# Modalities/modalities

Hardware: AMD Instinct MI355X
Metric: train_tokens_per_s (higher is better)
Workload: dtype bf16; 1 GPU; model=gpt2-2.7b, global_batch=2, micro_batch=2, seq_len=4096, parallelism=dp1_fullshard_hipgraph, num_params=2795276800

## Files before the change

### modalities_amd/ops/adamw.py

```python

from typing import Iterable

import torch

from modalities_amd.ops.backend import hip_ext, hip_available


@torch.no_grad()
def fused_adamw_step(params: list, grads: list, exp_avgs: list, exp_avg_sqs: list,
                     step: int, lr: float, beta1: float, beta2: float,
                     eps: float, weight_decay: float) -> None:
    bc1 = 1.0 - beta1 ** step
    bc2 = 1.0 - beta2 ** step
    if hip_available() and params and params[0].is_cuda:
        hip_ext().fused_adamw(params, grads, exp_avgs, exp_avg_sqs,
                              lr, beta1, beta2, eps, weight_decay, bc1, bc2)
        return
    for p, g, m, v in zip(params, grads, exp_avgs, exp_avg_sqs):
        p.mul_(1.0 - lr * weight_decay)
        m.mul_(beta1).add_(g, alpha=1 - beta1)
        v.mul_(beta2).addcmul_(g, g, value=1 - beta2)
        denom = (v / bc2).sqrt_().add_(eps)
        p.addcdiv_(m, denom, value=-lr / bc1)


@torch.no_grad()
def multi_tensor_l2norm(tensors: Iterable[torch.Tensor]) -> torch.Tensor:
    tensors = [t for t in tensors if t is not None]
    if not tensors:
        return torch.zeros((), dtype=torch.float32)
    if hip_available() and tensors[0].is_cuda:
        return hip_ext().multi_tensor_sqsum(list(tensors)).sqrt()
    acc = torch.zeros((), dtype=torch.float32, device=tensors[0].device)
    for t in tensors:
        acc += t.float().pow(2).sum()
    return acc.sqrt()


@torch.no_grad()
def multi_tensor_scale_(tensors: Iterable[torch.Tensor], scale: torch.Tensor) -> None:
    tensors = [t for t in tensors if t is not None]
    if not tensors:
        return
    if hip_available() and tensors[0].is_cuda and isinstance(scale, torch.Tensor):
        hip_ext().multi_tensor_scale(list(tensors), scale)
        return
    for t in tensors:
        t.mul_(scale.to(t.device) if isinstance(scale, torch.Tensor) else scale)
```

### modalities_amd/ops/csrc/adamw.hip

```cpp
#include <torch/extension.h>
#include <ATen/hip/HIPContext.h>
#include "common.h"

namespace {

__global__ void adamw_masked_kernel(float* __restrict__ p,
                                    const float* __restrict__ g,
                                    float* __restrict__ m,
                                    float* __restrict__ v,
                                    const float* __restrict__ wd_mask,
                                    long n4, float lr, float beta1, float beta2,
                                    float eps, float wd, float bc1, float bc2) {
  const float step_size = lr / bc1;
  const float inv_bc2 = 1.0f / bc2;
  floatx4* p4 = reinterpret_cast<floatx4*>(p);
  const floatx4* g4 = reinterpret_cast<const floatx4*>(g);
  floatx4* m4 = reinterpret_cast<floatx4*>(m);
  floatx4* v4 = reinterpret_cast<floatx4*>(v);
  const floatx4* w4 = reinterpret_cast<const floatx4*>(wd_mask);
  for (long i = blockIdx.x * (long)blockDim.x + threadIdx.x; i < n4;
       i += (long)gridDim.x * blockDim.x) {
    floatx4 pp = p4[i], gg = g4[i], mm = m4[i], vv = v4[i], ww = w4[i];
#pragma unroll
    for (int j = 0; j < 4; ++j) {
      pp[j] *= (1.0f - lr * wd * ww[j]);
      mm[j] = beta1 * mm[j] + (1.0f - beta1) * gg[j];
      vv[j] = beta2 * vv[j] + (1.0f - beta2) * gg[j] * gg[j];
      pp[j] -= step_size * mm[j] / (sqrtf(vv[j] * inv_bc2) + eps);
    }
    p4[i] = pp; m4[i] = mm; v4[i] = vv;
  }
}

__device__ __forceinline__ float bias_correction(float beta, float t) {
  return -expm1f(t * logf(beta));
}

__global__ void adamw_masked_devstep_kernel(float* __restrict__ p,
                                            const float* __restrict__ g,
                                            float* __restrict__ m,
                                            float* __restrict__ v,
                                            const float* __restrict__ wd_mask,
                                            const int* __restrict__ step,
                                            unsigned short* __restrict__ bf16_out,
                                            const float* __restrict__ gscale,
                                            long n4, float lr, float beta1,
                                            float beta2, float eps, float wd) {
  const float gs = gscale ? *gscale : 1.0f;
  const float t = (float)*step;
  const float bc1 = bias_correction(beta1, t);
  const float bc2 = bias_correction(beta2, t);
  const float step_size = lr / bc1;
  const float inv_bc2 = 1.0f / bc2;
  floatx4* p4 = reinterpret_cast<floatx4*>(p);
  const floatx4* g4 = reinterpret_cast<const floatx4*>(g);
  floatx4* m4 = reinterpret_cast<floatx4*>(m);
  floatx4* v4 = reinterpret_cast<floatx4*>(v);
  const floatx4* w4 = reinterpret_cast<const floatx4*>(wd_mask);
  for (long i = blockIdx.x * (long)blockDim.x + threadIdx.x; i < n4;
       i += (long)gridDim.x * blockDim.x) {
    floatx4 pp = p4[i], gg = g4[i], mm = m4[i], vv = v4[i], ww = w4[i];
    shortx4 h;
#pragma unroll
    for (int j = 0; j < 4; ++j) {
      const float gj = gg[j] * gs;
      pp[j] *= (1.0f - lr * wd * ww[j]);
      mm[j] = beta1 * mm[j] + (1.0f - beta1) * gj;
      vv[j] = beta2 * vv[j] + (1.0f - beta2) * gj * gj;
      pp[j] -= step_size * mm[j] / (sqrtf(vv[j] * inv_bc2) + eps);
      h[j] = (short)f32_to_bf16(pp[j]);
    }
    p4[i] = pp; m4[i] = mm; v4[i] = vv;
    reinterpret_cast<shortx4*>(bf16_out)[i] = h;
  }
}

template <int W>
__global__ void adamw_devstep_wide_kernel(float* __restrict__ p,
                                          const float* __restrict__ g,
                                          float* __restrict__ m,
                                          float* __restrict__ v,
                                          const float* __restrict__ wd_mask,
                                          const int* __restrict__ step,
                                          unsigned short* __restrict__ bf16_out,
                                          const float* __restrict__ gscale,
                                          long n4, float lr, float beta1,
                                          float beta2, float eps, float wd) {
  const float gs = gscale ? *gscale : 1.0f;
  const float t = (float)*step;
  const float bc1 = bias_correction(beta1, t);
  const float bc2 = bias_correction(beta2, t);
  const float step_size = lr / bc1;
  const float inv_bc2 = 1.0f / bc2;
  floatx4* p4 = reinterpret_cast<floatx4*>(p);
  const floatx4* g4 = reinterpret_cast<const floatx4*>(g);
  floatx4* m4 = reinterpret_cast<floatx4*>(m);
  floatx4* v4 = reinterpret_cast<floatx4*>(v);
  const floatx4* w4 = reinterpret_cast<const floatx4*>(wd_mask);
  const long stride = (long)gridDim.x * blockDim.x;
  for (long i0 = ((long)blockIdx.x * blockDim.x + threadIdx.x) * W;
       i0 < n4; i0 += stride * W) {
    floatx4 pp[W], gg[W], mm[W], vv[W], ww[W];
    shortx4 h[W];
#pragma unroll
    for (int u = 0; u < W; ++u)
      if (i0 + u < n4) {
        pp[u] = p4[i0 + u]; gg[u] = g4[i0 + u]; mm[u] = m4[i0 + u];
        vv[u] = v4[i0 + u]; ww[u] = w4[i0 + u];
      }
#pragma unroll
    for (int u = 0; u < W; ++u) {
#pragma unroll
      for (int j = 0; j < 4; ++j) {
        const float gj = gg[u][j] * gs;
        pp[u][j] *= (1.0f - lr * wd * ww[u][j]);
        mm[u][j] = beta1 * mm[u][j] + (1.0f - beta1) * gj;
        vv[u][j] = beta2 * vv[u][j] + (1.0f - beta2) * gj * gj;
        pp[u][j] -= step_size * mm[u][j] / (sqrtf(vv[u][j] * inv_bc2) + eps);
        h[u][j] = (short)f32_to_bf16(pp[u][j]);
      }
    }
#pragma unroll
    for (int u = 0; u < W; ++u)
      if (i0 + u < n4) {
        p4[i0 + u] = pp[u]; m4[i0 + u] = mm[u]; v4[i0 + u] = vv[u];
        reinterpret_cast<shortx4*>(bf16_out)[i0 + u] = h[u];
      }
  }
}

__global__ void sqsum_kernel(const float* __restrict__ x, long n4,
                             float* __restrict__ out) {
  __shared__ float scratch[256 / WAVE_SIZE];
  const floatx4* x4 = reinterpret_cast<const floatx4*>(x);
  float acc = 0.f;
  for (long i = blockIdx.x * (long)blockDim.x + threadIdx.x; i < n4;
       i += (long)gridDim.x * blockDim.x) {
    floatx4 v = x4[i];
#pragma unroll
    for (int j = 0; j < 4; ++j) acc += v[j] * v[j];
  }
  acc = block_reduce_sum(acc, scratch);
  if (threadIdx.x == 0) atomicAdd(out, acc);
}

__global__ void scale_kernel(float* __restrict__ x, long n4,
                             const float* __restrict__ scale) {
  const float s = *scale;
  floatx4* x4 = reinterpret_cast<floatx4*>(x);
  for (long i = blockIdx.x * (long)blockDim.x + threadIdx.x; i < n4;
       i += (long)gridDim.x * blockDim.x) {
    floatx4 v = x4[i];
#pragma unroll
    for (int j = 0; j < 4; ++j) v[j] *= s;
    x4[i] = v;
  }
}

int grid_for(long work, int block) {
  long g = (work + block - 1) / block;
  return (int)min(g, (long)(256 * 8));
}

bool f32_like(const torch::Tensor& t, const torch::Tensor& ref) {
  return t.is_cuda() && t.dtype() == torch::kFloat32 && t.is_contiguous()
      && t.numel() == ref.numel() && t.device() == ref.device();
}

}

void fused_adamw_masked(torch::Tensor p, torch::Tensor g, torch::Tensor m,
                        torch::Tensor v, torch::Tensor wd_mask, double lr,
                        double beta1, double beta2, double eps, double wd,
                        double bc1, double bc2) {
  TORCH_CHECK(p.is_cuda() && p.dtype() == torch::kFloat32 && p.is_contiguous());
  TORCH_CHECK(p.numel() % 4 == 0, "flat shard must be divisible by 4");
  TORCH_CHECK(f32_like(g, p) && f32_like(m, p) && f32_like(v, p)
              && f32_like(wd_mask, p),
              "g, m, v, wd_mask must match p (device fp32, contiguous)");
  long n4 = p.numel() / 4;
  auto stream = at::cuda::getCurrentHIPStream();
  hipLaunchKernelGGL(adamw_masked_kernel, dim3(grid_for(n4, 256)), dim3(256), 0,
                     stream, p.data_ptr<float>(), g.data_ptr<float>(),
                     m.data_ptr<float>(), v.data_ptr<float>(),
                     wd_mask.data_ptr<float>(), n4, (float)lr, (float)beta1,
                     (float)beta2, (float)eps, (float)wd, (float)bc1, (float)bc2);
  HIP_CHECK_KERNEL();
}

void fused_adamw_masked_devstep(torch::Tensor p, torch::Tensor g,
                                torch::Tensor m, torch::Tensor v,
                                torch::Tensor wd_mask, torch::Tensor step,
                                torch::Tensor bf16_out,
                                c10::optional<torch::Tensor> gscale, double lr,
                                double beta1, double beta2, double eps,
                                double wd) {
  const float* gs_ptr = nullptr;
  if (gscale.has_value()) {
    TORCH_CHECK(gscale->is_cuda() && gscale->dtype() == torch::kFloat32
                && gscale->numel() == 1, "gscale must be a cuda fp32 scalar");
    gs_ptr = gscale->data_ptr<float>();
  }
  TORCH_CHECK(p.is_cuda() && p.dtype() == torch::kFloat32 && p.is_contiguous());
  TORCH_CHECK(p.numel() % 4 == 0, "flat shard must be divisible by 4");
  TORCH_CHECK(f32_like(g, p) && f32_like(m, p) && f32_like(v, p)
              && f32_like(wd_mask, p),
              "g, m, v, wd_mask must match p (device fp32, contiguous)");
  TORCH_CHECK(step.is_cuda() && step.dtype() == torch::kInt32
              && step.numel() == 1);
  TORCH_CHECK(bf16_out.is_cuda() && bf16_out.dtype() == torch::kBFloat16
              && bf16_out.is_contiguous() && bf16_out.numel() == p.numel());
  long n4 = p.numel() / 4;
  auto stream = at::cuda::getCurrentHIPStream();
  static const int wide = []() {
    const char* e = getenv("MODALITIES_AMD_ADAMW_WIDE");
    return e ? atoi(e) : 1;
  }();
  if (wide >= 4) {
    hipLaunchKernelGGL(adamw_devstep_wide_kernel<4>,
                       dim3(grid_for((n4 + 3) / 4, 256)), dim3(256), 0, stream,
                       p.data_ptr<float>(), g.data_ptr<float>(),
                       m.data_ptr<float>(), v.data_ptr<float>(),
                       wd_mask.data_ptr<float>(), step.data_ptr<int>(),
                       (unsigned short*)bf16_out.data_ptr(), gs_ptr, n4,
                       (float)lr, (float)beta1, (float)beta2, (float)eps,
                       (float)wd);
  } else if (wide >= 2) {
    hipLaunchKernelGGL(adamw_devstep_wide_kernel<2>,
                       dim3(grid_for((n4 + 1) / 2, 256)), dim3(256), 0, stream,
                       p.data_ptr<float>(), g.data_ptr<float>(),
                       m.data_ptr<float>(), v.data_ptr<float>(),
                       wd_mask.data_ptr<float>(), step.data_ptr<int>(),
                       (unsigned short*)bf16_out.data_ptr(), gs_ptr, n4,
                       (float)lr, (float)beta1, (float)beta2, (float)eps,
                       (float)wd);
  } else {
    hipLaunchKernelGGL(adamw_masked_devstep_kernel, dim3(grid_for(n4, 256)),
                       dim3(256), 0, stream, p.data_ptr<float>(),
                       g.data_ptr<float>(), m.data_ptr<float>(),
                       v.data_ptr<float>(), wd_mask.data_ptr<float>(),
                       step.data_ptr<int>(),
                       (unsigned short*)bf16_out.data_ptr(), gs_ptr, n4,
                       (float)lr, (float)beta1, (float)beta2, (float)eps,
                       (float)wd);
  }
  HIP_CHECK_KERNEL();
}

void fused_adamw(std::vector<torch::Tensor> ps, std::vector<torch::Tensor> gs,
                 std::vector<torch::Tensor> ms, std::vector<torch::Tensor> vs,
                 double lr, double beta1, double beta2, double eps, double wd,
                 double bc1, double bc2) {
  TORCH_CHECK(gs.size() == ps.size() && ms.size() == ps.size()
              && vs.size() == ps.size(), "fused_adamw: list lengths differ");
  for (size_t i = 0; i < ps.size(); ++i) {
    auto ones = torch::ones_like(ps[i]);
    fused_adamw_masked(ps[i], gs[i], ms[i], vs[i], ones, lr, beta1, beta2, eps,
                       wd, bc1, bc2);
  }
}

torch::Tensor multi_tensor_sqsum(std::vector<torch::Tensor> tensors) {
  TORCH_CHECK(!tensors.empty());
  auto out = torch::zeros({}, tensors[0].options().dtype(torch::kFloat32));
  auto stream = at::cuda::getCurrentHIPStream();
  for (auto& t : tensors) {
    TORCH_CHECK(t.is_cuda() && t.dtype() == torch::kFloat32
                && t.is_contiguous() && t.numel() % 4 == 0);
    long n4 = t.numel() / 4;
    hipLaunchKernelGGL(sqsum_kernel, dim3(grid_for(n4, 256)), dim3(256), 0,
                       stream, t.data_ptr<float>(), n4, out.data_ptr<float>());
    HIP_CHECK_KERNEL();
  }
  return out;
}

void multi_tensor_scale(std::vector<torch::Tensor> tensors, torch::Tensor scale) {
  TORCH_CHECK(scale.is_cuda() && scale.numel() == 1,
              "multi_tensor_scale: scale must be a device scalar");
  for (auto& t : tensors)
    TORCH_CHECK(t.is_cuda() && t.dtype() == torch::kFloat32
                && t.is_contiguous() && t.numel() % 4 == 0,
                "multi_tensor_scale: tensors must be contiguous device fp32 "
                "with numel % 4 == 0");
  auto stream = at::cuda::getCurrentHIPStream();
  auto s = scale.to(torch::kFloat32).contiguous();
  for (auto& t : tensors) {
    long n4 = t.numel() / 4;
    hipLaunchKernelGGL(scale_kernel, dim3(grid_for(n4, 256)), dim3(256), 0,
                       stream, t.data_ptr<float>(), n4, s.data_ptr<float>());
    HIP_CHECK_KERNEL();
  }
}
```

### modalities_amd/ops/csrc/bindings.cpp

```cpp
#include <torch/extension.h>

std::vector<torch::Tensor> rmsnorm_fwd(torch::Tensor x, torch::Tensor w, double eps);
std::vector<torch::Tensor> rmsnorm_bwd(torch::Tensor dy, torch::Tensor x,
                                       torch::Tensor w, torch::Tensor invrms);
std::vector<torch::Tensor> layernorm_fwd(torch::Tensor x, torch::Tensor w,
                                         c10::optional<torch::Tensor> b,
                                         double eps);
std::vector<torch::Tensor> layernorm_bwd(torch::Tensor dy, torch::Tensor x,
                                         torch::Tensor w, torch::Tensor mean,
                                         torch::Tensor rstd, bool has_bias);
long layernorm_max_h();
torch::Tensor rope_fwd(torch::Tensor x, torch::Tensor cos_t, torch::Tensor sin_t,
                       bool neg);
torch::Tensor rope_fwd_slice(torch::Tensor qkv, torch::Tensor cos_t,
                             torch::Tensor sin_t, long col_off, long Hn,
                             long D, bool neg);
void rope_bwd_slice(torch::Tensor dx, torch::Tensor cos_t, torch::Tensor sin_t,
                    torch::Tensor dqkv, long col_off);
torch::Tensor silu_mul_fwd(torch::Tensor g, torch::Tensor u);
std::vector<torch::Tensor> silu_mul_bwd(torch::Tensor dout, torch::Tensor g,
                                        torch::Tensor u);
torch::Tensor silu_mul_joint_fwd(torch::Tensor wv);
torch::Tensor silu_mul_joint_bwd(torch::Tensor dout, torch::Tensor wv);
std::vector<torch::Tensor> cross_entropy_fwd(torch::Tensor logits,
                                             torch::Tensor targets,
                                             long ignore_index);
torch::Tensor cross_entropy_bwd(torch::Tensor logits, torch::Tensor targets,
                                torch::Tensor lse, torch::Tensor scale,
                                long ignore_index);
void fused_adamw_masked(torch::Tensor p, torch::Tensor g, torch::Tensor m,
                        torch::Tensor v, torch::Tensor wd_mask, double lr,
                        double beta1, double beta2, double eps, double wd,
                        double bc1, double bc2);
void fused_adamw_masked_devstep(torch::Tensor p, torch::Tensor g,
                                torch::Tensor m, torch::Tensor v,
                                torch::Tensor wd_mask, torch::Tensor step,
                                torch::Tensor bf16_out,
                                c10::optional<torch::Tensor> gscale, double lr,
                                double beta1, double beta2, double eps,
                                double wd);
void fused_adamw(std::vector<torch::Tensor> ps, std::vector<torch::Tensor> gs,
                 std::vector<torch::Tensor> ms, std::vector<torch::Tensor> vs,
                 double lr, double beta1, double beta2, double eps, double wd,
                 double bc1, double bc2);
torch::Tensor multi_tensor_sqsum(std::vector<torch::Tensor> tensors);
void multi_tensor_scale(std::vector<torch::Tensor> tensors, torch::Tensor scale);
std::vector<torch::Tensor> attn_fwd(torch::Tensor q, torch::Tensor k,
                                    torch::Tensor v, bool causal,
                                    long q_offset);
std::vector<torch::Tensor> attn_bwd(torch::Tensor dout, torch::Tensor q,
                                    torch::Tensor k, torch::Tensor v,
                                    torch::Tensor o, torch::Tensor lse,
                                    bool causal, long q_offset,
                                    c10::optional<torch::Tensor> dlse);
torch::Tensor mfma_probe_32x32x16(torch::Tensor a, torch::Tensor b);
torch::Tensor tr16_probe(long mode);
std::vector<torch::Tensor> attn_fwd_ablate(torch::Tensor q, torch::Tensor k,
                                           torch::Tensor v, long mode);
std::vector<torch::Tensor> attn_bwd_qkvjoint(torch::Tensor dout,
                                             torch::Tensor q, torch::Tensor k,
                                             torch::Tensor v, torch::Tensor o,
                                             torch::Tensor lse, bool causal,
                                             long q_offset, torch::Tensor dqkv,
                                             long dv_col_off);
std::vector<torch::Tensor> attn_bwd_dkdv_ablate(torch::Tensor dout,
                                                torch::Tensor q,
                                                torch::Tensor k,
                                                torch::Tensor v,
                                                torch::Tensor lse,
                                                torch::Tensor delta, long mode);
std::vector<torch::Tensor> attn_fwd2(torch::Tensor q, torch::Tensor k,
                                     torch::Tensor v, bool causal,
                                     long q_offset);
std::vector<torch::Tensor> attn_bwd2(torch::Tensor dout, torch::Tensor q,
                                     torch::Tensor k, torch::Tensor v,
                                     torch::Tensor o, torch::Tensor lse,
                                     bool causal, long q_offset,
                                     c10::optional<torch::Tensor> dlse);
std::vector<torch::Tensor> attn_bwd2_qkvjoint(torch::Tensor dout,
                                              torch::Tensor q, torch::Tensor k,
                                              torch::Tensor v, torch::Tensor o,
                                              torch::Tensor lse, bool causal,
                                              long q_offset, torch::Tensor dqkv,
                                              long dv_col_off);
std::vector<torch::Tensor> attn_fwd2_doc(torch::Tensor q, torch::Tensor k,
                                         torch::Tensor v, bool causal,
                                         long q_offset,
                                         torch::Tensor doc_start);
std::vector<torch::Tensor> attn_bwd2_doc(torch::Tensor dout, torch::Tensor q,
                                         torch::Tensor k, torch::Tensor v,
                                         torch::Tensor o, torch::Tensor lse,
                                         bool causal, long q_offset,
                                         torch::Tensor doc_start,
                                         torch::Tensor doc_end,
                                         c10::optional<torch::Tensor> dlse);
std::vector<torch::Tensor> attn_bwd2_qkvjoint_doc(
    torch::Tensor dout, torch::Tensor q, torch::Tensor k, torch::Tensor v,
    torch::Tensor o, torch::Tensor lse, bool causal, long q_offset,
    torch::Tensor doc_start, torch::Tensor doc_end, torch::Tensor dqkv,
    long dv_col_off);
std::vector<torch::Tensor> decode_attn_fwd(torch::Tensor q,
                                           torch::Tensor k_cache,
                                           torch::Tensor v_cache,
                                           torch::Tensor kv_lens,
                                           long kv_chunk);
long decode_attn_kv_chunk();
long decode_attn_kv_chunk_min();
torch::Tensor decode_rope_append(torch::Tensor q, torch::Tensor k,
                                 torch::Tensor v,
                                 c10::optional<torch::Tensor> cos_t,
                                 c10::optional<torch::Tensor> sin_t,
                                 torch::Tensor pos, torch::Tensor k_cache,
                                 torch::Tensor v_cache);

static int g_attn_impl = [] {
  const char* e = getenv("MA_ATTN_IMPL");
  return e ? atoi(e) : 2;
}();

PYBIND11_MODULE(TORCH_EXTENSION_NAME, m) {
  m.def("rmsnorm_fwd", &rmsnorm_fwd, "RMSNorm forward (K5)");
  m.def("rmsnorm_bwd", &rmsnorm_bwd, "RMSNorm backward (K5)");
  m.def("layernorm_fwd", &layernorm_fwd,
        "LayerNorm forward (K5): (y, mean, rstd); b may be None",
        py::arg("x"), py::arg("w"), py::arg("b"), py::arg("eps"));
  m.def("layernorm_bwd", &layernorm_bwd,
        "LayerNorm backward (K5): (dx, dw, db); db is empty without bias",
        py::arg("dy"), py::arg("x"), py::arg("w"), py::arg("mean"),
        py::arg("rstd"), py::arg("has_bias"));
  m.def("layernorm_max_h", &layernorm_max_h,
        "largest row length the LayerNorm kernels take");
  m.def("rope_fwd", &rope_fwd, "RoPE rotate-half (K4); neg=true => inverse");
  m.def("rope_fwd_slice", &rope_fwd_slice,
        "RoPE a head-block slice of fused QKV into a contiguous [B,T,H,D]");
  m.def("rope_bwd_slice", &rope_bwd_slice,
        "inverse-RoPE a [B,T,H,D] grad into a fused-QKV grad buffer slice");
  m.def("silu_mul_fwd", &silu_mul_fwd, "silu(g)*u forward (K6)");
  m.def("silu_mul_bwd", &silu_mul_bwd, "silu(g)*u backward (K6)");
  m.def("silu_mul_joint_fwd", &silu_mul_joint_fwd,
        "silu/mul over a packed [.., 2H] gate|up tensor (K6 joint)");
  m.def("silu_mul_joint_bwd", &silu_mul_joint_bwd,
        "joint-layout silu/mul backward into one dwv buffer");
  m.def("cross_entropy_fwd", &cross_entropy_fwd, "fused CE forward (K8)");
  m.def("cross_entropy_bwd", &cross_entropy_bwd, "fused CE backward (K8)");
  m.def("fused_adamw_masked", &fused_adamw_masked,
        "AdamW on a flat fp32 shard with per-element wd mask (K9)");
  m.def("fused_adamw", &fused_adamw, "multi-tensor AdamW (K9)");
  m.def("fused_adamw_masked_devstep", &fused_adamw_masked_devstep,
        "AdamW with device-resident step counter (hipGraph-safe)");
  m.def("multi_tensor_sqsum", &multi_tensor_sqsum, "sum of squares (K10)");
  m.def("multi_tensor_scale", &multi_tensor_scale, "in-place scale (K10)");
  m.def("attn_fwd",
        [](torch::Tensor q, torch::Tensor k, torch::Tensor v, bool causal,
           long q_offset) {
          const long D = q.size(3);
          return (g_attn_impl == 2 || D == 80)
              ? attn_fwd2(q, k, v, causal, q_offset)
              : attn_fwd(q, k, v, causal, q_offset);
        },
        "flash attention forward (K1)", py::arg("q"), py::arg("k"),
        py::arg("v"), py::arg("causal"), py::arg("q_offset") = 0);
  m.def("attn_bwd",
        [](torch::Tensor dout, torch::Tensor q, torch::Tensor k,
           torch::Tensor v, torch::Tensor o, torch::Tensor lse, bool causal,
           long q_offset, c10::optional<torch::Tensor> dlse) {
          const long D = q.size(3);
          return (g_attn_impl == 2 || D == 80)
              ? attn_bwd2(dout, q, k, v, o, lse, causal, q_offset, dlse)
              : attn_bwd(dout, q, k, v, o, lse, causal, q_offset, dlse);
        },
        "flash attention backward (K1); dlse = d(loss)/d(lse) fp32 [B,Hq,T] "
        "or None", py::arg("dout"), py::arg("q"),
        py::arg("k"), py::arg("v"), py::arg("o"), py::arg("lse"),
        py::arg("causal"), py::arg("q_offset") = 0,
        py::arg("dlse") = py::none());
  m.def("set_attn_impl", [](long v) { g_attn_impl = (int)v; },
        "select the K1 kernel generation (1 or 2) for A/B");
  m.def("get_attn_impl", []() { return (long)g_attn_impl; });
  m.def("attn_fwd_v1", &attn_fwd, "K1 v1 forward (direct, for A/B)");
  m.def("attn_bwd_v1", &attn_bwd, "K1 v1 backward (direct, for A/B)",
        py::arg("dout"), py::arg("q"), py::arg("k"), py::arg("v"),
        py::arg("o"), py::arg("lse"), py::arg("causal"), py::arg("q_offset"),
        py::arg("dlse") = py::none());
  m.def("attn_fwd_v2", &attn_fwd2, "K1 v2 forward (direct, for A/B)");
  m.def("attn_bwd_v2", &attn_bwd2, "K1 v2 backward (direct, for A/B)",
        py::arg("dout"), py::arg("q"), py::arg("k"), py::arg("v"),
        py::arg("o"), py::arg("lse"), py::arg("causal"), py::arg("q_offset"),
        py::arg("dlse") = py::none());
  m.def("tr16_probe", &tr16_probe, "ds_read_b64_tr_b16 semantics probe");
  m.def("mfma_probe_32x32x16", &mfma_probe_32x32x16,
        "MFMA fragment-layout probe (verification)");
  m.def("attn_fwd_ablate", &attn_fwd_ablate,
        "attention fwd cost-attribution ablation (timing only)");
  m.def("attn_bwd_qkvjoint",
        [](torch::Tensor dout, torch::Tensor q, torch::Tensor k,
           torch::Tensor v, torch::Tensor o, torch::Tensor lse, bool causal,
           long q_offset, torch::Tensor dqkv, long dv_col_off) {
          const long D = q.size(3);
          return (g_attn_impl == 2 || D == 80)
              ? attn_bwd2_qkvjoint(dout, q, k, v, o, lse, causal, q_offset,
                                   dqkv, dv_col_off)
              : attn_bwd_qkvjoint(dout, q, k, v, o, lse, causal, q_offset,
                                  dqkv, dv_col_off);
// ... 73 lines not shown
```

### modalities_amd/optimizers/optimizer_factory.py

```python

from typing import Optional

import torch

from modalities_amd.parallel.fsdp import XGMIShardedModel


class ShardedAdamW(torch.optim.Optimizer):

    def __init__(self, sharded_model: XGMIShardedModel, lr: float = 3e-4,
                 betas: tuple[float, float] = (0.9, 0.95), eps: float = 1e-8,
                 weight_decay: float = 0.1):
        self.sharded_model = sharded_model
        sharded_model._optimizer_consumes_grad_scale = True
        sharded_model._pending_grad_scale = None
        params = [u.master_shard for u in sharded_model.units]
        defaults = dict(lr=lr, betas=betas, eps=eps, weight_decay=weight_decay)
        super().__init__(params, defaults)
        for u in sharded_model.units:
            st = self.state[u.master_shard]
            st["step"] = 0
            st["exp_avg"] = torch.zeros_like(u.master_shard)
            st["exp_avg_sq"] = torch.zeros_like(u.master_shard)
        self._step_dev = None

    @torch.no_grad()
    def step(self, closure=None):
        loss = closure() if closure is not None else None
        group = self.param_groups[0]
        lr, (beta1, beta2) = group["lr"], group["betas"]
        eps, wd = group["eps"], group["weight_decay"]
        from modalities_amd.ops.backend import hip_available, hip_ext
        on_gpu = hip_available() and self.sharded_model.units \
            and self.sharded_model.units[0].master_shard.is_cuda
        if on_gpu:
            if self._step_dev is None:
                start = max((self.state[u.master_shard].get("step", 0)
                             for u in self.sharded_model.units), default=0)
                self._step_dev = torch.tensor(
                    start, dtype=torch.int32,
                    device=self.sharded_model.units[0].master_shard.device)
            self._step_dev += 1
            fresh = [u.grad_fresh for u in self.sharded_model.units]
            if any(fresh) and not all(fresh):
                raise RuntimeError(
                    "fused AdamW devstep: mixed grad_fresh across units "
                    f"({sum(fresh)}/{len(fresh)}) — the shared device step "
                    "counter requires all units to step together")
        gscale = getattr(self.sharded_model, "_pending_grad_scale", None)
        self.sharded_model._pending_grad_scale = None
        for ui, u in enumerate(self.sharded_model.units):
            if not u.grad_fresh:
                continue
            st = self.state[u.master_shard]
            st["step"] += 1
            step = st["step"]
            m, v = st["exp_avg"], st["exp_avg_sq"]
            g = u.grad_shard
            p = u.master_shard
            if on_gpu and u.bf16_shard.dtype == torch.bfloat16:
                hip_ext().fused_adamw_masked_devstep(
                    p, g, m, v, u.wd_mask_shard, self._step_dev,
                    u.bf16_shard, gscale, lr, beta1, beta2, eps, wd)
                if u.full_buf is not None and self.sharded_model.world > 1:
                    u.free_full()
                self.sharded_model.prefetch_unit_gather(ui)
            elif on_gpu:
                if gscale is not None:
                    g = g.mul(gscale)
                bc1 = 1.0 - beta1 ** step
                bc2 = 1.0 - beta2 ** step
                hip_ext().fused_adamw_masked(p, g, m, v, u.wd_mask_shard,
                                             lr, beta1, beta2, eps, wd,
                                             bc1, bc2)
                u.publish_master()
            else:
                if gscale is not None:
                    g = g.mul(gscale)
                bc1 = 1.0 - beta1 ** step
                bc2 = 1.0 - beta2 ** step
                p.mul_(1.0 - lr * wd * u.wd_mask_shard)
                m.mul_(beta1).add_(g, alpha=1 - beta1)
                v.mul_(beta2).addcmul_(g, g, value=1 - beta2)
                denom = (v / bc2).sqrt().add_(eps)
                p.add_(-lr / bc1 * m / denom)
        if on_gpu:
            pass
        else:
            self.sharded_model.publish_master()
            for ui in range(len(self.sharded_model.units)):
                self.sharded_model.prefetch_unit_gather(ui)
        return loss

    def zero_grad(self, set_to_none: bool = True):
        self.sharded_model.zero_grad_shards()


def get_adam_w(wrapped_model, lr: float = 3e-4, betas=(0.9, 0.95), eps: float = 1e-8,
               weight_decay: float = 0.1, weight_decay_groups_excluded=None,
               foreach: Optional[bool] = None, fused: Optional[bool] = None):
    if isinstance(wrapped_model, XGMIShardedModel):
        return ShardedAdamW(wrapped_model, lr=lr, betas=betas, eps=eps,
                            weight_decay=weight_decay)
    decay, no_decay = [], []
    for name, p in wrapped_model.named_parameters():
        if not p.requires_grad:
            continue
        (no_decay if p.ndim < 2 or "norm" in name.lower() or name.endswith(".bias")
         else decay).append(p)
    groups = [{"params": decay, "weight_decay": weight_decay},
              {"params": no_decay, "weight_decay": 0.0}]
    return torch.optim.AdamW(groups, lr=lr, betas=betas, eps=eps,
# ... 2 lines not shown
```

### modalities_amd/parallel/fsdp.py

```python

import re
from contextlib import contextmanager
from typing import Optional

import torch
import torch.distributed as dist
import torch.nn as nn


def _pad_to(n: int, multiple: int) -> int:
    return (n + multiple - 1) // multiple * multiple


class _CommStreams:
    def __init__(self, device: torch.device):
        self.on_gpu = device.type == "cuda"
        self.gather = torch.cuda.Stream(device=device) if self.on_gpu else None
        self.reduce = torch.cuda.Stream(device=device) if self.on_gpu else None

    @contextmanager
    def on(self, stream):
        if self.on_gpu and stream is not None:
            with torch.cuda.stream(stream):
                yield
        else:
            yield


class FlatParamUnit:

    def __init__(self, name: str, modules: list[nn.Module], device: torch.device,
                 group, rank: int, world: int, param_dtype: torch.dtype,
                 no_decay_patterns: Optional[list[str]] = None):
        self.name = name
        self.modules = modules
        self.device = device
        self.group = group
        self.rank = rank
        self.world = world
        self.param_dtype = param_dtype

        seen: dict[int, int] = {}
        self.param_infos: list[tuple[nn.Module, str, nn.Parameter]] = []
        for mod in modules:
            for pname, p in mod.named_parameters(recurse=True):
                if id(p) in seen:
                    continue
                seen[id(p)] = len(self.param_infos)
                self.param_infos.append((mod, pname, p))

        self.shapes = [p.shape for _, _, p in self.param_infos]
        self.numels = [p.numel() for _, _, p in self.param_infos]
        self.offsets = []
        off = 0
        for n in self.numels:
            self.offsets.append(off)
            off += n
        self.total_numel = _pad_to(max(off, 1), max(world, 1) * 64)
        self.shard_numel = self.total_numel // world

        nd_res = [re.compile(pat) for pat in (no_decay_patterns or [])]
        flat_mask = torch.ones(self.total_numel, dtype=torch.float32)
        for (mod, pname, p), offset, numel in zip(self.param_infos, self.offsets,
                                                  self.numels):
            full_name = f"{type(mod).__name__}.{pname}"
            no_decay = p.ndim < 2 or any(r.search(full_name) for r in nd_res)
            if no_decay:
                flat_mask[offset:offset + numel] = 0.0
        s = self.rank * self.shard_numel
        self.wd_mask_shard = flat_mask[s:s + self.shard_numel].to(device)

        self.master_shard = torch.zeros(self.shard_numel, dtype=torch.float32, device=device)
        self.grad_shard = torch.empty(self.shard_numel, dtype=torch.float32, device=device)
        self.grad_fresh = False
        self.bf16_shard = torch.zeros(self.shard_numel, dtype=param_dtype, device=device)
        self.full_buf: Optional[torch.Tensor] = None
        self.grad_full: Optional[torch.Tensor] = None
        self.is_gathered = False
        self.grads_allocated = False
        self.grads_seen = 0
        self._gather_event = None
        self._reduce_event = None


    @torch.no_grad()
    def init_from_materialized(self):
        flat = torch.zeros(self.total_numel, dtype=torch.float32, device=self.device)
        for (_, _, p), off, n in zip(self.param_infos, self.offsets, self.numels):
            flat[off:off + n] = p.detach().float().reshape(-1).to(self.device)
        s = self.rank * self.shard_numel
        self.master_shard.copy_(flat[s:s + self.shard_numel])
        self.bf16_shard.copy_(self.master_shard.to(self.param_dtype))
        del flat
        self._point_params_to(None)

    @torch.no_grad()
    def _point_params_to(self, full_buf: Optional[torch.Tensor]):
        for (_, _, p), off, n, shape in zip(self.param_infos, self.offsets,
                                            self.numels, self.shapes):
            if full_buf is None:
                p.data = torch.empty(0, dtype=self.param_dtype, device=self.device)
            else:
                p.data = full_buf[off:off + n].view(shape)


    def gather(self, streams: _CommStreams):
        if self.is_gathered:
            return
        if self.world == 1:
            self.full_buf = self.bf16_shard
            self.is_gathered = True
            return
        with streams.on(streams.gather):
            if streams.on_gpu:
                streams.gather.wait_stream(torch.cuda.current_stream(self.device))
            self.full_buf = torch.empty(self.total_numel, dtype=self.param_dtype,
                                        device=self.device)
            dist.all_gather_into_tensor(self.full_buf, self.bf16_shard, group=self.group)
            if streams.on_gpu:
                self._gather_event = torch.cuda.Event()
                self._gather_event.record(streams.gather)
        self.is_gathered = True

    def wait_gather(self, streams: _CommStreams):
        if streams.on_gpu and self._gather_event is not None:
            torch.cuda.current_stream(self.device).wait_event(self._gather_event)
            self._gather_event = None
            if self.full_buf is not None and self.full_buf.is_cuda:
                self.full_buf.record_stream(
                    torch.cuda.current_stream(self.device))
        self._point_params_to(self.full_buf)

    @torch.no_grad()
    def free_full(self):
        self._point_params_to(None)
        self.full_buf = None
        self.is_gathered = False


    @torch.no_grad()
    def alloc_grad_views(self):
        if self.grad_full is None:
            self.grad_full = torch.zeros(self.total_numel, dtype=self.param_dtype,
                                         device=self.device)
        for (_, _, p), off, n, shape in zip(self.param_infos, self.offsets,
                                            self.numels, self.shapes):
            p.grad = self.grad_full[off:off + n].view(shape)
        self.grads_allocated = True

    def reduce_scatter_grads(self, streams: _CommStreams):
        gf = self.grad_full
        if gf is None:
            return
        with streams.on(streams.reduce):
            if streams.on_gpu:
                streams.reduce.wait_stream(torch.cuda.current_stream(self.device))
            if self.world > 1:
                backend = dist.get_backend(self.group) if self.group is not None \
                    else dist.get_backend()
                if backend != "gloo":
                    out = torch.empty(self.shard_numel, dtype=self.param_dtype,
                                      device=self.device)
                    dist.reduce_scatter_tensor(out, gf, group=self.group)
                else:
                    dist.all_reduce(gf, group=self.group)
                    s = self.rank * self.shard_numel
                    out = gf[s:s + self.shard_numel]
            else:
                out = gf
            scale = 1.0 / self.world
            if self.grad_fresh:
                self.grad_shard.add_(out, alpha=scale)
            else:
                self.grad_shard.copy_(out)
                if scale != 1.0:
                    self.grad_shard.mul_(scale)
                self.grad_fresh = True
            if streams.on_gpu:
                self._reduce_event = torch.cuda.Event()
                self._reduce_event.record(streams.reduce)
                gf.record_stream(streams.reduce)
        for _, _, p in self.param_infos:
            p.grad = None
        self.grad_full = None
        self.grads_allocated = False

    def wait_reduce(self):
        if self._reduce_event is not None:
            torch.cuda.current_stream(self.device).wait_event(self._reduce_event)
            self._reduce_event = None

    @torch.no_grad()
    def publish_master(self):
        self.bf16_shard.copy_(self.master_shard)
        if self.world > 1 and self.full_buf is not None:
            self.free_full()


class _UnshardBackwardAnchor(torch.autograd.Function):

    @staticmethod
    def forward(ctx, engine, unit_idx, t):
        ctx.engine = engine
        ctx.unit_idx = unit_idx
        return t.view_as(t)

    @staticmethod
    def backward(ctx, grad):
        ctx.engine._pre_backward(ctx.unit_idx)
        return None, None, grad


class XGMIShardedModel(nn.Module):

    def __init__(self, module: nn.Module, device: torch.device,
                 process_group=None, rank: Optional[int] = None,
                 world_size: Optional[int] = None,
                 unit_modules: Optional[list[list[nn.Module]]] = None,
                 param_dtype: torch.dtype = torch.bfloat16,
                 reshard_after_forward: bool = False,
                 no_decay_patterns: Optional[list[str]] = None,
                 replicate_group=None):
        super().__init__()
        self.module = module
        self.device = device
        self.group = process_group
        if world_size is None:
            world_size = dist.get_world_size(process_group) if dist.is_initialized() else 1
        if rank is None:
# ... 100 lines not shown

    def _prefetch_after(self, idx):
        try:
            pos = self._known_order.index(idx)
            nxt = self._known_order[pos + 1]
        except (ValueError, IndexError):
            return
        self.units[nxt].gather(self.streams)


    def _pre_backward(self, idx):
        unit = self.units[idx]
        if not unit.is_gathered:
            unit.gather(self.streams)
            try:
                pos = self._known_order.index(idx)
                if pos > 0 and self.reshard_after_forward:
                    self.units[self._known_order[pos - 1]].gather(self.streams)
            except ValueError:
                pass
        unit.wait_gather(self.streams)
        if not unit.grads_allocated:
            unit.alloc_grad_views()

    def _finish_unit_backward(self, idx):
        self._units_needing_reduce.discard(idx)
        unit = self.units[idx]
        unit.reduce_scatter_grads(self.streams)
        if self.reshard_after_forward:
            unit.free_full()


    def forward(self, *args, **kwargs):
        if self._fwd_order:
            self._known_order = list(self._fwd_order)
        self._fwd_order = []
        for u in self.units:
            u.grads_seen = 0
        if not self.reshard_after_forward:
            for u in self.units:
                if not u.is_gathered:
                    u.gather(self.streams)
        return self.module(*args, **kwargs)

    def backward_epilogue(self):
        for idx in list(self._units_needing_reduce):
            self._finish_unit_backward(idx)
        for u in self.units:
            u.wait_reduce()
            u.grads_seen = 0
        if self._replicate_group is not None:
            ws = dist.get_world_size(self._replicate_group)
            for u in self.units:
                dist.all_reduce(u.grad_shard, group=self._replicate_group)
                u.grad_shard.div_(ws)

    @torch.no_grad()
    def zero_grad_shards(self):
        for u in self.units:
            u.grad_fresh = False

    @torch.no_grad()
    def publish_master(self):
        for u in self.units:
            u.publish_master()

    @torch.no_grad()
    def prefetch_unit_gather(self, idx: int):
        if self.reshard_after_forward or self.world == 1:
            return
        u = self.units[idx]
        if not u.is_gathered:
            u.gather(self.streams)

    @torch.no_grad()
    def free_stale_fulls(self):
        if self.world > 1:
            for u in self.units:
                if u.full_buf is not None:
                    u.free_full()

    @torch.no_grad()
    def clip_grad_norm_(self, max_norm: Optional[float],
                        norm_type: float = 2.0,
                        pp_group=None) -> torch.Tensor:
        from modalities_amd.ops.adamw import multi_tensor_l2norm, multi_tensor_scale_
        fresh = [u.grad_shard for u in self.units if u.grad_fresh]
        local = multi_tensor_l2norm(fresh) ** 2
        if local.device != torch.device(self.device):
            local = local.to(self.device)
        if self.world > 1:
            dist.all_reduce(local, group=self.group)
        if pp_group is not None:
            dist.all_reduce(local, group=pp_group)
        total = local.sqrt()
        if max_norm is not None and max_norm > 0 and fresh:
            clip = (max_norm / (total + 1e-6)).clamp(max=1.0)
            if getattr(self, "_optimizer_consumes_grad_scale", False) \
                    and total.is_cuda:
                self._pending_grad_scale = clip
            else:
                multi_tensor_scale_(fresh, clip)
        return total


    def shard_state_dict(self) -> dict[str, torch.Tensor]:
        return {f"{u.name}.master_shard": u.master_shard for u in self.units}

    def load_shard_state_dict(self, sd: dict):
        for u in self.units:
            u.master_shard.copy_(sd[f"{u.name}.master_shard"])
            u.publish_master()

    def shard_meta(self) -> dict:
        return {
            u.name: {
                "total_numel": u.total_numel,
                "params": [
                    {"module": type(mod).__name__, "name": pname,
                     "offset": off, "numel": n, "shape": list(shape)}
                    for (mod, pname, _), off, n, shape in
                    zip(u.param_infos, u.offsets, u.numels, u.shapes)
                ],
            }
            for u in self.units
        }

    @torch.no_grad()
    def gather_full_state_dict(self) -> dict[str, torch.Tensor]:
        name_of = {}
        for name, p in self.module.named_parameters():
            name_of[id(p)] = name
        out = {}
        for u in self.units:
            full = torch.empty(u.total_numel, dtype=torch.float32, device=self.device)
            if self.world > 1:
                dist.all_gather_into_tensor(full, u.master_shard, group=self.group)
            else:
                full.copy_(u.master_shard)
            for (mod, pname, p), off, n, shape in zip(u.param_infos, u.offsets,
                                                      u.numels, u.shapes):
                key = name_of.get(id(p), f"{u.name}:{pname}")
                out[key] = full[off:off + n].view(shape).clone()
        return out
```

Before: 33720 tokens/s.

## Feed bf16 reduced grads and bit-packed decay mask directly into AdamW

The reduced gradient is no longer copied and upcast into an fp32 grad shard. Instead the bf16 reduce output is kept as a pending grad, and the AdamW and grad-norm kernels read it directly, applying the scale factor inside the kernel. The fp32 weight-decay mask is replaced by a bit-packed uint8 mask, which cuts the optimizer's memory traffic per element. The cost is extra lazy-materialization logic, a stream lifetime dependency on the reduce output, and removal of the wide-kernel variants.

```diff
diff --git a/modalities_amd/ops/adamw.py b/modalities_amd/ops/adamw.py
--- a/modalities_amd/ops/adamw.py
+++ b/modalities_amd/ops/adamw.py
@@ -25,6 +25,17 @@
 
 
 @torch.no_grad()
+def pack_wd_bits(mask: torch.Tensor):
+    assert mask.numel() % 8 == 0, "mask length must be a multiple of 8"
+    if not bool(((mask == 0) | (mask == 1)).all()):
+        return None
+    weights = torch.tensor([1, 2, 4, 8, 16, 32, 64, 128], dtype=torch.int32,
+                           device=mask.device)
+    bits = ((mask != 0).reshape(-1, 8).to(torch.int32) * weights).sum(1)
+    return bits.to(torch.uint8)
+
+
+@torch.no_grad()
 def multi_tensor_l2norm(tensors: Iterable[torch.Tensor]) -> torch.Tensor:
     tensors = [t for t in tensors if t is not None]
     if not tensors:
diff --git a/modalities_amd/ops/csrc/adamw.hip b/modalities_amd/ops/csrc/adamw.hip
--- a/modalities_amd/ops/csrc/adamw.hip
+++ b/modalities_amd/ops/csrc/adamw.hip
@@ -36,16 +36,43 @@
   return -expm1f(t * logf(beta));
 }
 
-__global__ void adamw_masked_devstep_kernel(float* __restrict__ p,
-                                            const float* __restrict__ g,
-                                            float* __restrict__ m,
-                                            float* __restrict__ v,
-                                            const float* __restrict__ wd_mask,
-                                            const int* __restrict__ step,
-                                            unsigned short* __restrict__ bf16_out,
-                                            const float* __restrict__ gscale,
-                                            long n4, float lr, float beta1,
-                                            float beta2, float eps, float wd) {
+__device__ __forceinline__ floatx4 load_grad4(const float* g, long i, float) {
+  return reinterpret_cast<const floatx4*>(g)[i];
+}
+
+__device__ __forceinline__ floatx4 load_grad4(const unsigned short* g, long i,
+                                              float gmul) {
+  const shortx4 h = reinterpret_cast<const shortx4*>(g)[i];
+  floatx4 r;
+#pragma unroll
+  for (int j = 0; j < 4; ++j) r[j] = bf16_to_f32((unsigned short)h[j]) * gmul;
+  return r;
+}
+
+__device__ __forceinline__ floatx4 load_mask4(const float* w, long i) {
+  return reinterpret_cast<const floatx4*>(w)[i];
+}
+
+__device__ __forceinline__ floatx4 load_mask4(const unsigned char* bits,
+                                              long i) {
+  const unsigned b = (unsigned)bits[i >> 1] >> ((unsigned)(i & 1) * 4u);
+  floatx4 r;
+#pragma unroll
+  for (int j = 0; j < 4; ++j) r[j] = ((b >> j) & 1u) ? 1.0f : 0.0f;
+  return r;
+}
+
+template <typename G, typename W>
+__global__ void adamw_devstep_kernel(float* __restrict__ p,
+                                     const G* __restrict__ g, float gmul,
+                                     float* __restrict__ m,
+                                     float* __restrict__ v,
+                                     const W* __restrict__ wd_mask,
+                                     const int* __restrict__ step,
+                                     unsigned short* __restrict__ bf16_out,
+                                     const float* __restrict__ gscale,
+                                     long n4, float lr, float beta1,
+                                     float beta2, float eps, float wd) {
   const float gs = gscale ? *gscale : 1.0f;
   const float t = (float)*step;
   const float bc1 = bias_correction(beta1, t);
@@ -53,13 +80,13 @@
   const float step_size = lr / bc1;
   const float inv_bc2 = 1.0f / bc2;
   floatx4* p4 = reinterpret_cast<floatx4*>(p);
-  const floatx4* g4 = reinterpret_cast<const floatx4*>(g);
   floatx4* m4 = reinterpret_cast<floatx4*>(m);
   floatx4* v4 = reinterpret_cast<floatx4*>(v);
-  const floatx4* w4 = reinterpret_cast<const floatx4*>(wd_mask);
   for (long i = blockIdx.x * (long)blockDim.x + threadIdx.x; i < n4;
        i += (long)gridDim.x * blockDim.x) {
-    floatx4 pp = p4[i], gg = g4[i], mm = m4[i], vv = v4[i], ww = w4[i];
+    floatx4 pp = p4[i], mm = m4[i], vv = v4[i];
+    const floatx4 gg = load_grad4(g, i, gmul);
+    const floatx4 ww = load_mask4(wd_mask, i);
     shortx4 h;
 #pragma unroll
     for (int j = 0; j < 4; ++j) {
@@ -75,68 +102,14 @@
   }
 }
 
-template <int W>
-__global__ void adamw_devstep_wide_kernel(float* __restrict__ p,
-                                          const float* __restrict__ g,
-                                          float* __restrict__ m,
-                                          float* __restrict__ v,
-                                          const float* __restrict__ wd_mask,
-                                          const int* __restrict__ step,
-                                          unsigned short* __restrict__ bf16_out,
-                                          const float* __restrict__ gscale,
-                                          long n4, float lr, float beta1,
-                                          float beta2, float eps, float wd) {
-  const float gs = gscale ? *gscale : 1.0f;
-  const float t = (float)*step;
-  const float bc1 = bias_correction(beta1, t);
-  const float bc2 = bias_correction(beta2, t);
-  const float step_size = lr / bc1;
-  const float inv_bc2 = 1.0f / bc2;
-  floatx4* p4 = reinterpret_cast<floatx4*>(p);
-  const floatx4* g4 = reinterpret_cast<const floatx4*>(g);
-  floatx4* m4 = reinterpret_cast<floatx4*>(m);
-  floatx4* v4 = reinterpret_cast<floatx4*>(v);
-  const floatx4* w4 = reinterpret_cast<const floatx4*>(wd_mask);
-  const long stride = (long)gridDim.x * blockDim.x;
-  for (long i0 = ((long)blockIdx.x * blockDim.x + threadIdx.x) * W;
-       i0 < n4; i0 += stride * W) {
-    floatx4 pp[W], gg[W], mm[W], vv[W], ww[W];
-    shortx4 h[W];
-#pragma unroll
-    for (int u = 0; u < W; ++u)
-      if (i0 + u < n4) {
-        pp[u] = p4[i0 + u]; gg[u] = g4[i0 + u]; mm[u] = m4[i0 + u];
-        vv[u] = v4[i0 + u]; ww[u] = w4[i0 + u];
-      }
-#pragma unroll
-    for (int u = 0; u < W; ++u) {
-#pragma unroll
-      for (int j = 0; j < 4; ++j) {
-        const float gj = gg[u][j] * gs;
-        pp[u][j] *= (1.0f - lr * wd * ww[u][j]);
-        mm[u][j] = beta1 * mm[u][j] + (1.0f - beta1) * gj;
-        vv[u][j] = beta2 * vv[u][j] + (1.0f - beta2) * gj * gj;
-        pp[u][j] -= step_size * mm[u][j] / (sqrtf(vv[u][j] * inv_bc2) + eps);
-        h[u][j] = (short)f32_to_bf16(pp[u][j]);
-      }
-    }
-#pragma unroll
-    for (int u = 0; u < W; ++u)
-      if (i0 + u < n4) {
-        p4[i0 + u] = pp[u]; m4[i0 + u] = mm[u]; v4[i0 + u] = vv[u];
-        reinterpret_cast<shortx4*>(bf16_out)[i0 + u] = h[u];
-      }
-  }
-}
-
-__global__ void sqsum_kernel(const float* __restrict__ x, long n4,
+template <typename G>
+__global__ void sqsum_kernel(const G* __restrict__ x, float gmul, long n4,
                              float* __restrict__ out) {
   __shared__ float scratch[256 / WAVE_SIZE];
-  const floatx4* x4 = reinterpret_cast<const floatx4*>(x);
   float acc = 0.f;
   for (long i = blockIdx.x * (long)blockDim.x + threadIdx.x; i < n4;
        i += (long)gridDim.x * blockDim.x) {
-    floatx4 v = x4[i];
+    floatx4 v = load_grad4(x, i, gmul);
 #pragma unroll
     for (int j = 0; j < 4; ++j) acc += v[j] * v[j];
   }
@@ -165,6 +138,13 @@
 bool f32_like(const torch::Tensor& t, const torch::Tensor& ref) {
   return t.is_cuda() && t.dtype() == torch::kFloat32 && t.is_contiguous()
       && t.numel() == ref.numel() && t.device() == ref.device();
+}
+
+const float* gscale_ptr(const c10::optional<torch::Tensor>& gscale) {
+  if (!gscale.has_value()) return nullptr;
+  TORCH_CHECK(gscale->is_cuda() && gscale->dtype() == torch::kFloat32
+              && gscale->numel() == 1, "gscale must be a cuda fp32 scalar");
+  return gscale->data_ptr<float>();
 }
 
 }
@@ -195,12 +175,7 @@
                                 c10::optional<torch::Tensor> gscale, double lr,
                                 double beta1, double beta2, double eps,
                                 double wd) {
-  const float* gs_ptr = nullptr;
-  if (gscale.has_value()) {
-    TORCH_CHECK(gscale->is_cuda() && gscale->dtype() == torch::kFloat32
-                && gscale->numel() == 1, "gscale must be a cuda fp32 scalar");
-    gs_ptr = gscale->data_ptr<float>();
-  }
+  const float* gs_ptr = gscale_ptr(gscale);
   TORCH_CHECK(p.is_cuda() && p.dtype() == torch::kFloat32 && p.is_contiguous());
   TORCH_CHECK(p.numel() % 4 == 0, "flat shard must be divisible by 4");
   TORCH_CHECK(f32_like(g, p) && f32_like(m, p) && f32_like(v, p)
@@ -212,38 +187,53 @@
               && bf16_out.is_contiguous() && bf16_out.numel() == p.numel());
   long n4 = p.numel() / 4;
   auto stream = at::cuda::getCurrentHIPStream();
-  static const int wide = []() {
-    const char* e = getenv("MODALITIES_AMD_ADAMW_WIDE");
-    return e ? atoi(e) : 1;
-  }();
-  if (wide >= 4) {
-    hipLaunchKernelGGL(adamw_devstep_wide_kernel<4>,
-                       dim3(grid_for((n4 + 3) / 4, 256)), dim3(256), 0, stream,
-                       p.data_ptr<float>(), g.data_ptr<float>(),
-                       m.data_ptr<float>(), v.data_ptr<float>(),
-                       wd_mask.data_ptr<float>(), step.data_ptr<int>(),
-                       (unsigned short*)bf16_out.data_ptr(), gs_ptr, n4,
-                       (float)lr, (float)beta1, (float)beta2, (float)eps,
-                       (float)wd);
-  } else if (wide >= 2) {
-    hipLaunchKernelGGL(adamw_devstep_wide_kernel<2>,
-                       dim3(grid_for((n4 + 1) / 2, 256)), dim3(256), 0, stream,
-                       p.data_ptr<float>(), g.data_ptr<float>(),
-                       m.data_ptr<float>(), v.data_ptr<float>(),
-                       wd_mask.data_ptr<float>(), step.data_ptr<int>(),
-                       (unsigned short*)bf16_out.data_ptr(), gs_ptr, n4,
-                       (float)lr, (float)beta1, (float)beta2, (float)eps,
-                       (float)wd);
-  } else {
-    hipLaunchKernelGGL(adamw_masked_devstep_kernel, dim3(grid_for(n4, 256)),
-                       dim3(256), 0, stream, p.data_ptr<float>(),
-                       g.data_ptr<float>(), m.data_ptr<float>(),
-                       v.data_ptr<float>(), wd_mask.data_ptr<float>(),
-                       step.data_ptr<int>(),
-                       (unsigned short*)bf16_out.data_ptr(), gs_ptr, n4,
-                       (float)lr, (float)beta1, (float)beta2, (float)eps,
-                       (float)wd);
-  }
+  hipLaunchKernelGGL((adamw_devstep_kernel<float, float>),
+                     dim3(grid_for(n4, 256)), dim3(256), 0, stream,
+                     p.data_ptr<float>(), g.data_ptr<float>(), 1.0f,
+                     m.data_ptr<float>(), v.data_ptr<float>(),
+                     wd_mask.data_ptr<float>(), step.data_ptr<int>(),
+                     (unsigned short*)bf16_out.data_ptr(), gs_ptr, n4,
+                     (float)lr, (float)beta1, (float)beta2, (float)eps,
+                     (float)wd);
+  HIP_CHECK_KERNEL();
+}
+
+void fused_adamw_devstep_bf16g(torch::Tensor p, torch::Tensor g, double gmul,
+                               torch::Tensor m, torch::Tensor v,
+                               torch::Tensor wd_bits, torch::Tensor step,
+                               torch::Tensor bf16_out,
+                               c10::optional<torch::Tensor> gscale, double lr,
+                               double beta1, double beta2, double eps,
+                               double wd) {
+  const float* gs_ptr = gscale_ptr(gscale);
+  TORCH_CHECK(p.is_cuda() && p.dtype() == torch::kFloat32 && p.is_contiguous());
+  TORCH_CHECK(p.numel() % 8 == 0,
+              "flat shard must be divisible by 8 (one mask byte per 8)");
+  TORCH_CHECK(f32_like(m, p) && f32_like(v, p),
+              "m, v must match p (device fp32, contiguous)");
+  TORCH_CHECK(g.is_cuda() && g.dtype() == torch::kBFloat16 && g.is_contiguous()
+              && g.numel() == p.numel() && g.device() == p.device(),
+              "g must be a contiguous device bf16 tensor of p's size");
+  TORCH_CHECK(wd_bits.is_cuda() && wd_bits.dtype() == torch::kUInt8
+              && wd_bits.is_contiguous() && wd_bits.numel() * 8 == p.numel()
+              && wd_bits.device() == p.device(),
+              "wd_bits must be a contiguous device uint8 tensor of "
+              "p.numel() / 8 bytes");
+  TORCH_CHECK(step.is_cuda() && step.dtype() == torch::kInt32
+              && step.numel() == 1);
+  TORCH_CHECK(bf16_out.is_cuda() && bf16_out.dtype() == torch::kBFloat16
+              && bf16_out.is_contiguous() && bf16_out.numel() == p.numel());
+  long n4 = p.numel() / 4;
+  auto stream = at::cuda::getCurrentHIPStream();
+  hipLaunchKernelGGL((adamw_devstep_kernel<unsigned short, unsigned char>),
+                     dim3(grid_for(n4, 256)), dim3(256), 0, stream,
+                     p.data_ptr<float>(),
+                     (const unsigned short*)g.data_ptr(), (float)gmul,
+                     m.data_ptr<float>(), v.data_ptr<float>(),
+                     wd_bits.data_ptr<unsigned char>(), step.data_ptr<int>(),
+                     (unsigned short*)bf16_out.data_ptr(), gs_ptr, n4,
+                     (float)lr, (float)beta1, (float)beta2, (float)eps,
+                     (float)wd);
   HIP_CHECK_KERNEL();
 }
 
@@ -268,8 +258,31 @@
     TORCH_CHECK(t.is_cuda() && t.dtype() == torch::kFloat32
                 && t.is_contiguous() && t.numel() % 4 == 0);
     long n4 = t.numel() / 4;
-    hipLaunchKernelGGL(sqsum_kernel, dim3(grid_for(n4, 256)), dim3(256), 0,
-                       stream, t.data_ptr<float>(), n4, out.data_ptr<float>());
+    hipLaunchKernelGGL(sqsum_kernel<float>, dim3(grid_for(n4, 256)), dim3(256),
+                       0, stream, t.data_ptr<float>(), 1.0f, n4,
+                       out.data_ptr<float>());
+    HIP_CHECK_KERNEL();
+  }
+  return out;
+}
+
+torch::Tensor multi_tensor_sqsum_bf16(std::vector<torch::Tensor> tensors,
+                                      double gmul) {
+  TORCH_CHECK(!tensors.empty());
+  for (auto& t : tensors)
+    TORCH_CHECK(t.is_cuda() && t.dtype() == torch::kBFloat16
+                && t.is_contiguous() && t.numel() % 8 == 0
+                && t.device() == tensors[0].device(),
+                "multi_tensor_sqsum_bf16: tensors must be contiguous device "
+                "bf16 with numel % 8 == 0");
+  auto out = torch::zeros({}, tensors[0].options().dtype(torch::kFloat32));
+  auto stream = at::cuda::getCurrentHIPStream();
+  for (auto& t : tensors) {
+    long n4 = t.numel() / 4;
+    hipLaunchKernelGGL(sqsum_kernel<unsigned short>, dim3(grid_for(n4, 256)),
+                       dim3(256), 0, stream,
+                       (const unsigned short*)t.data_ptr(), (float)gmul, n4,
+                       out.data_ptr<float>());
     HIP_CHECK_KERNEL();
   }
   return out;
diff --git a/modalities_amd/ops/csrc/bindings.cpp b/modalities_amd/ops/csrc/bindings.cpp
--- a/modalities_amd/ops/csrc/bindings.cpp
+++ b/modalities_amd/ops/csrc/bindings.cpp
@@ -44,6 +44,15 @@
                  double lr, double beta1, double beta2, double eps, double wd,
                  double bc1, double bc2);
 torch::Tensor multi_tensor_sqsum(std::vector<torch::Tensor> tensors);
+void fused_adamw_devstep_bf16g(torch::Tensor p, torch::Tensor g, double gmul,
+                               torch::Tensor m, torch::Tensor v,
+                               torch::Tensor wd_bits, torch::Tensor step,
+                               torch::Tensor bf16_out,
+                               c10::optional<torch::Tensor> gscale, double lr,
+                               double beta1, double beta2, double eps,
+                               double wd);
+torch::Tensor multi_tensor_sqsum_bf16(std::vector<torch::Tensor> tensors,
+                                      double gmul);
 void multi_tensor_scale(std::vector<torch::Tensor> tensors, torch::Tensor scale);
 std::vector<torch::Tensor> attn_fwd(torch::Tensor q, torch::Tensor k,
                                     torch::Tensor v, bool causal,
@@ -149,6 +158,11 @@
   m.def("fused_adamw_masked_devstep", &fused_adamw_masked_devstep,
         "AdamW with device-resident step counter (hipGraph-safe)");
   m.def("multi_tensor_sqsum", &multi_tensor_sqsum, "sum of squares (K10)");
+  m.def("fused_adamw_devstep_bf16g", &fused_adamw_devstep_bf16g,
+        "device-step AdamW reading a bf16 grad (* gmul) and a bit-packed "
+        "decay mask (K9)");
+  m.def("multi_tensor_sqsum_bf16", &multi_tensor_sqsum_bf16,
+        "sum of squares of float(bf16) * gmul (K10)");
   m.def("multi_tensor_scale", &multi_tensor_scale, "in-place scale (K10)");
   m.def("attn_fwd",
         [](torch::Tensor q, torch::Tensor k, torch::Tensor v, bool causal,
diff --git a/modalities_amd/optimizers/optimizer_factory.py b/modalities_amd/optimizers/optimizer_factory.py
--- a/modalities_amd/optimizers/optimizer_factory.py
+++ b/modalities_amd/optimizers/optimizer_factory.py
@@ -23,6 +23,20 @@
             st["exp_avg"] = torch.zeros_like(u.master_shard)
             st["exp_avg_sq"] = torch.zeros_like(u.master_shard)
         self._step_dev = None
+        self._wd_bits = {}
+        for u in sharded_model.units:
+            if u.keep_bf16_grads:
+                self._wd_bits_for(u)
+
+    def _wd_bits_for(self, u):
+        from modalities_amd.ops.adamw import pack_wd_bits
+        mask = u.wd_mask_shard
+        cached = self._wd_bits.get(u.name)
+        if cached is None or cached[1] is not mask \
+                or cached[2] != mask._version:
+            cached = (pack_wd_bits(mask), mask, mask._version)
+            self._wd_bits[u.name] = cached
+        return cached[0]
 
     @torch.no_grad()
     def step(self, closure=None):
@@ -56,8 +70,19 @@
             st["step"] += 1
             step = st["step"]
             m, v = st["exp_avg"], st["exp_avg_sq"]
+            p = u.master_shard
+            bits = self._wd_bits_for(u) if on_gpu \
+                and u._pending_grad is not None else None
+            if bits is not None:
+                hip_ext().fused_adamw_devstep_bf16g(
+                    p, u._pending_grad, u._pending_gmul, m, v, bits,
+                    self._step_dev, u.bf16_shard, gscale, lr, beta1, beta2,
+                    eps, wd)
+                if u.full_buf is not None and self.sharded_model.world > 1:
+                    u.free_full()
+                self.sharded_model.prefetch_unit_gather(ui)
+                continue
             g = u.grad_shard
-            p = u.master_shard
             if on_gpu and u.bf16_shard.dtype == torch.bfloat16:
                 hip_ext().fused_adamw_masked_devstep(
                     p, g, m, v, u.wd_mask_shard, self._step_dev,
diff --git a/modalities_amd/parallel/fsdp.py b/modalities_amd/parallel/fsdp.py
--- a/modalities_amd/parallel/fsdp.py
+++ b/modalities_amd/parallel/fsdp.py
@@ -1,4 +1,5 @@
 
+import os
 import re
 from contextlib import contextmanager
 from typing import Optional
@@ -71,8 +72,14 @@
         self.wd_mask_shard = flat_mask[s:s + self.shard_numel].to(device)
 
         self.master_shard = torch.zeros(self.shard_numel, dtype=torch.float32, device=device)
-        self.grad_shard = torch.empty(self.shard_numel, dtype=torch.float32, device=device)
+        self._grad_shard_f32 = torch.empty(self.shard_numel, dtype=torch.float32,
+                                           device=device)
         self.grad_fresh = False
+        self.keep_bf16_grads = (
+            device.type == "cuda" and param_dtype == torch.bfloat16
+            and os.environ.get("MODALITIES_AMD_BF16_GRAD_PATH", "1") != "0")
+        self._pending_grad: Optional[torch.Tensor] = None
+        self._pending_gmul = 1.0
         self.bf16_shard = torch.zeros(self.shard_numel, dtype=param_dtype, device=device)
         self.full_buf: Optional[torch.Tensor] = None
         self.grad_full: Optional[torch.Tensor] = None
@@ -81,6 +88,27 @@
         self.grads_seen = 0
         self._gather_event = None
         self._reduce_event = None
+
+
+    @property
+    def grad_shard(self) -> torch.Tensor:
+        self.materialize_grad()
+        return self._grad_shard_f32
+
+    @grad_shard.setter
+    def grad_shard(self, value: torch.Tensor):
+        self._pending_grad = None
+        self._grad_shard_f32 = value
+
+    @torch.no_grad()
+    def materialize_grad(self):
+        out = self._pending_grad
+        if out is None:
+            return
+        self._pending_grad = None
+        self._grad_shard_f32.copy_(out)
+        if self._pending_gmul != 1.0:
+            self._grad_shard_f32.mul_(self._pending_gmul)
 
 
     @torch.no_grad()
@@ -152,6 +180,8 @@
         gf = self.grad_full
         if gf is None:
             return
+        compute = torch.cuda.current_stream(self.device) if streams.on_gpu \
+            else None
         with streams.on(streams.reduce):
             if streams.on_gpu:
                 streams.reduce.wait_stream(torch.cuda.current_stream(self.device))
@@ -172,9 +202,12 @@
             if self.grad_fresh:
                 self.grad_shard.add_(out, alpha=scale)
             else:
-                self.grad_shard.copy_(out)
-                if scale != 1.0:
-                    self.grad_shard.mul_(scale)
+                self._pending_grad, self._pending_gmul = out, scale
+                if self.keep_bf16_grads:
+                    if out is not gf:
+                        out.record_stream(compute)
+                else:
+                    self.materialize_grad()
                 self.grad_fresh = True
             if streams.on_gpu:
                 self._reduce_event = torch.cuda.Event()
@@ -381,13 +414,15 @@
         if self._replicate_group is not None:
             ws = dist.get_world_size(self._replicate_group)
             for u in self.units:
-                dist.all_reduce(u.grad_shard, group=self._replicate_group)
-                u.grad_shard.div_(ws)
+                g = u.grad_shard
+                dist.all_reduce(g, group=self._replicate_group)
+                g.div_(ws)
 
     @torch.no_grad()
     def zero_grad_shards(self):
         for u in self.units:
             u.grad_fresh = False
+            u._pending_grad = None
 
     @torch.no_grad()
     def publish_master(self):
@@ -414,8 +449,22 @@
                         norm_type: float = 2.0,
                         pp_group=None) -> torch.Tensor:
         from modalities_amd.ops.adamw import multi_tensor_l2norm, multi_tensor_scale_
-        fresh = [u.grad_shard for u in self.units if u.grad_fresh]
-        local = multi_tensor_l2norm(fresh) ** 2
+        units = [u for u in self.units if u.grad_fresh]
+        clipping = max_norm is not None and max_norm > 0
+        defer = getattr(self, "_optimizer_consumes_grad_scale", False)
+        if clipping and not defer:
+            for u in units:
+                u.materialize_grad()
+        pending = [u for u in units if u._pending_grad is not None]
+        fresh = [u.grad_shard for u in units if u._pending_grad is None]
+        if pending:
+            from modalities_amd.ops.backend import hip_ext
+            local = hip_ext().multi_tensor_sqsum_bf16(
+                [u._pending_grad for u in pending], pending[0]._pending_gmul)
+            if fresh:
+                local = local + multi_tensor_l2norm(fresh) ** 2
+        else:
+            local = multi_tensor_l2norm(fresh) ** 2
         if local.device != torch.device(self.device):
             local = local.to(self.device)
         if self.world > 1:
@@ -423,10 +472,9 @@
         if pp_group is not None:
             dist.all_reduce(local, group=pp_group)
         total = local.sqrt()
-        if max_norm is not None and max_norm > 0 and fresh:
+        if clipping and units:
             clip = (max_norm / (total + 1e-6)).clamp(max=1.0)
-            if getattr(self, "_optimizer_consumes_grad_scale", False) \
-                    and total.is_cuda:
+            if defer and total.is_cuda:
                 self._pending_grad_scale = clip
             else:
                 multi_tensor_scale_(fresh, clip)
```

Result: faster. 34650 tokens/s, median of 6 (+2.8%).
